# blepping/ComfyUI-sonar

Measured on AMD Instinct MI355X. Metric: noise-latents/sec (SDXL 4x128x128), higher is better.
Workload: dtype f32

## Files before the change

comfyui-sonar_amd/csrc/plan.hip:

```cpp
#include <math.h>
#include <string.h>

#include <memory>
#include <type_traits>
#include <utility>
#include <vector>

#include "common.h"

namespace sonar {
namespace {

template <typename T>
inline T word_to(uint64_t w) {
    if constexpr (std::is_pointer_v<T>) {
        return reinterpret_cast<T>(static_cast<uintptr_t>(w));
    } else if constexpr (std::is_same_v<T, float>) {
        const uint32_t lo = (uint32_t)w;
        float f;
        memcpy(&f, &lo, sizeof f);
        return f;
    } else if constexpr (std::is_same_v<T, double>) {
        double d;
        memcpy(&d, &w, sizeof d);
// ... 42 lines not shown
    SONAR_REPLAYABLE(sonar_philox_normal_chain_f32),
    SONAR_REPLAYABLE(sonar_perlin_lattice_f32),
    SONAR_REPLAYABLE(sonar_perlin_generate_f32),
    SONAR_REPLAYABLE(sonar_perlin_generate_acc_f32),
    SONAR_REPLAYABLE(sonar_perlin_generate_chain_f32),
    SONAR_REPLAYABLE(sonar_perlin_noise_f32),
    SONAR_REPLAYABLE(sonar_perlin_noise_ahead_f32),
    SONAR_REPLAYABLE(sonar_pyramid_generate_f32),
    SONAR_REPLAYABLE(sonar_pyramid_generate_acc_f32),
    SONAR_REPLAYABLE(sonar_pyramid_generate_acc_ahead_f32),
    SONAR_REPLAYABLE(sonar_pyramid_noise_f32),
    SONAR_REPLAYABLE(sonar_pyramid_noise_ahead_f32),
    SONAR_REPLAYABLE(sonar_power_noise_f32),
    SONAR_REPLAYABLE(sonar_power_block_f32),
    SONAR_REPLAYABLE(sonar_power_noise_ahead_f32),
    SONAR_REPLAYABLE(sonar_power_irfft2_f32),
    SONAR_REPLAYABLE(sonar_spectral_filter_f32),
    SONAR_REPLAYABLE(sonar_channel_mix_f32),
    SONAR_REPLAYABLE(sonar_std_scale_f32),
    SONAR_REPLAYABLE(sonar_powerlaw_f32),
    SONAR_REPLAYABLE(sonar_mul_table_f32),
    SONAR_REPLAYABLE(sonar_stats_finalize),
    SONAR_REPLAYABLE(sonar_scale_noise_rows_f32),
    SONAR_REPLAYABLE(sonar_blend_f32),
    SONAR_REPLAYABLE(sonar_blend_tensor_f32),
    SONAR_REPLAYABLE(sonar_scalar_op_f32),
    SONAR_REPLAYABLE(sonar_rowstats_f32),
    SONAR_REPLAYABLE(sonar_row_affine_f32),
    SONAR_REPLAYABLE(sonar_amax_mid_f32),
    SONAR_REPLAYABLE(sonar_div_mid_f32),
// ... 208 lines not shown
```

comfyui-sonar_amd/csrc/power_core.h:

```cpp
#pragma once
#include <math.h>
#include <stdlib.h>

#include <type_traits>

#include "common.h"
#include "twiddles256.h"

namespace sonar {

using c32 = float2;

typedef float v2f __attribute__((ext_vector_type(2)));
__device__ __forceinline__ v2f vv(c32 a) { return v2f{a.x, a.y}; }
__device__ __forceinline__ c32 cc(v2f a) { return make_float2(a.x, a.y); }
__device__ __forceinline__ c32 cadd(c32 a, c32 b) { return cc(vv(a) + vv(b)); }
__device__ __forceinline__ c32 csub(c32 a, c32 b) { return cc(vv(a) - vv(b)); }
__device__ __forceinline__ c32 cmul(c32 a, c32 b) {
    const v2f A = vv(a), B = vv(b);
    return cc(__builtin_elementwise_fma(A.yy, v2f{-B.y, B.x}, A.xx * B));
}
__device__ __forceinline__ c32 cadd_i(c32 a, c32 b) { return cc(__builtin_elementwise_fma(vv(b).yx, v2f{-1.0f, 1.0f}, vv(a))); }
__device__ __forceinline__ c32 csub_i(c32 a, c32 b) { return cc(__builtin_elementwise_fma(vv(b).yx, v2f{1.0f, -1.0f}, vv(a))); }
__device__ __forceinline__ c32 cmul_i(c32 a) { return cc(vv(a).yx * v2f{-1.0f, 1.0f}); }
// ... 292 lines not shown
constexpr int kStatsBatch = 4;
struct StatsAhead {
    double* partials = nullptr;
    uint64_t stream_id = 0;
    int main_blocks = 0;
};
template <int H, int W>
__device__ __forceinline__ void power_stats_body(const float* __restrict__ filter, int64_t planes, uint64_t seed, uint64_t stream_id,
                                                 int64_t plane_offset, int group, int split, double* partials, int64_t bid, int64_t nb,
                                                 c32 (*EDGE)[2][H], double* red);

struct Ahead {
    int have_stats = 0;
    uint64_t next_stream = 0;
    double* next = nullptr;
};


}
```

comfyui-sonar_amd/csrc/power_fft.hip:

```cpp
#include "power_core.h"

namespace sonar {

template <int H, int W>
constexpr int plane_min_waves() {
    return (H * W >= 32768 || (H == 256 && W == 64) || (H == 64 && W == 256) || (H == 64 && W == 32)) ? 2 : 4;
}

template <int H, int W, int SRC, bool STATS, bool NORM>
__global__ void __launch_bounds__((plane_threads<H, W>()), (plane_min_waves<H, W>())) power_irfft2_kernel(const float* __restrict__ z,
                                                                       const float* __restrict__ filter, float* out,
                                                                       int64_t planes, uint64_t seed, uint64_t stream_id,
                                                                       int64_t plane_offset, int group, int split, double* partials,
                                                                       NormArgs na, StatsAhead sa) {
    kernarg_touch_for(z, filter, out, planes, seed, stream_id, plane_offset, group, split, partials, na, sa);
    using C = PlaneCfg<H, W>;
    constexpr int NT = plane_threads<H, W>();
    constexpr int M = C::M, S = C::S;
    constexpr int RN1 = C::RN1, RN2 = C::RN2;
    constexpr bool FAST = (W == 128) && (H == 128 || H == 64) && (NT == 512);
    constexpr int CN1 = FAST ? H / 8 : C::CN1, CN2 = FAST ? 8 : C::CN2;
    __shared__ c32 A[C::kLdsComplex];
    c32* const T0 = A + H * S;
    c32* const TM = T0 + H;
// ... 1021 lines not shown
            }
            partials_next[2 * slot] = ss;
            partials_next[2 * slot + 1] = qq;
        }
    }
};

template <int IT0, int IT1, int N>
__device__ __forceinline__ void pin_chunk(c32 (&v)[N]) {
#pragma unroll
    for (int it = IT0; it < IT1; ++it) {
        asm volatile("" : "+v"(v[it].x), "+v"(v[it].y), "+v"(v[it + N / 2].x), "+v"(v[it + N / 2].y));
    }
}

template <int H, int W, bool STATS, bool NORM>
__global__ void __launch_bounds__(1024) power_pipe_kernel(const float* __restrict__ filter, float* out, int64_t planes, uint64_t seed,
                                                          uint64_t stream_id, int64_t plane_offset, int group, int split, double* partials,
                                                          NormArgs na, uint64_t next_stream, double* partials_next) {
    kernarg_touch_for(filter, out, planes, seed, stream_id, plane_offset, group, split, partials, na, next_stream, partials_next);
    using C = PlaneCfg<H, W>;
    constexpr int NT = 512, NALL = 1024;
    static_assert(plane_threads<H, W>() == NT && W == 128 && H == 128, "one 8-wave team per plane, slot = one radix-16 column item");
    constexpr int M = C::M, S = C::S, Wh = M + 1, RN1 = C::RN1, RN2 = C::RN2, CN1 = H / 8, CN2 = 8, ITER = draw_iters<H, W>();
    constexpr int LM = draw_shift<W>();
    constexpr int E0 = kPipeChunks[0], E1 = E0 + kPipeChunks[1];
    static_assert(E1 <= ITER && ITER == CN1 / 2, "chunks of whole pair iterations");
    constexpr int BUF = H * S;
    __shared__ c32 PLANES[2 * BUF];
    __shared__ c32 EDGE[3 * H];
    __shared__ uint4 SEED_RT[NT];
    static_assert(sizeof(uint4) * NT >= sizeof(c32) * 2 * H * kAheadMaxGroup, "edge columns of a look-ahead unit fit the seed area");
    __shared__ double sred[2 * NT / 64];
    __shared__ double red[2 * NALL / 64];
// ... 245 lines not shown
                    gp = 0;
                    unit += gridDim.x;
                }
            }
            SONAR_PIPE_STAMP(3);
            __syncthreads();
        }
    }
    if (ahead) {
        __syncthreads();
        if (drawer && my_units == 2) TeamStats<H, W>::store(sred, tid, partials_next, (int64_t)blockIdx.x + gridDim.x);
    }
    if constexpr (STATS) write_partial<NALL>(s, q, partials, red);
}

template <int H, int W>
__device__ __forceinline__ void power_stats_body(const float* __restrict__ filter, int64_t planes, uint64_t seed, uint64_t stream_id,
                                                 int64_t plane_offset, int group, int split, double* partials, int64_t bid, int64_t nb,
                                                 c32 (*EDGE)[2][H] , double* red) {
    constexpr int NT = plane_threads<H, W>(), M = W / 2, Wh = M + 1;
    constexpr int NB = kStatsBatch;
    const int tid = threadIdx.x;
    double s = 0.0, q = 0.0;
    auto edge_terms = [&](int p) {
        float edge = 0.0f;
        for (int ky = tid; ky < H; ky += NT) {
            const int kn = (H - ky) & (H - 1);
            const c32 a = EDGE[p][0][ky], an = EDGE[p][0][kn], b = EDGE[p][1][ky], bn = EDGE[p][1][kn];
            const float ar = 0.5f * (a.x + an.x), ai = 0.5f * (a.y - an.y), br = 0.5f * (b.x + bn.x), bi = 0.5f * (b.y - bn.y);
            edge += (ar * ar + ai * ai) + (br * br + bi * bi);
// ... 86 lines not shown
template <int H, int W>
static int power_grid(int64_t planes, bool owns_partials = true) {
    using C = PlaneCfg<H, W>;
    static_assert(C::kLdsBytes + 256 <= 160 * 1024, "plane does not fit in LDS");
    const int threads_cu = H >= 128 ? 1024 : 2048;
    const int per_cu = (int)std::max<size_t>(1, std::min<size_t>(threads_cu / plane_threads<H, W>(), (160 * 1024) / (C::kLdsBytes + 256)));
    const int64_t g = std::min<int64_t>(planes, (int64_t)256 * per_cu);
    return (int)(owns_partials ? std::min<int64_t>(g, kNPart) : g);
}

static int& pipe_switch() {
    static int on = [] { const char* e = getenv("SONAR_POWER_PIPE"); return (e && e[0] == '0') ? 0 : 1; }();
    return on;
}
static bool pipe_enabled() { return pipe_switch() != 0; }
static int64_t pipe_units(int64_t planes, int group, int* psplit) {
    *psplit = group > 1 && planes / group < 256 ? 1 : 0;
    return *psplit ? planes : planes / group;
}

template <int H, int W>
static int launch_power(int what, const float* z, const float* filter, float* out, int64_t planes, uint64_t seed,
                        uint64_t stream_id, int64_t plane_offset, int group, double* partials, NormArgs na, hipStream_t st,
                        Ahead ah = Ahead()) {
    if constexpr (H == 128 && W == 128) {
        if (pipe_enabled() && z == nullptr && (what == 0 || what == 1) && planes > 256) {
            int psplit;
            const int64_t units = pipe_units(planes, group, &psplit);
            const int pg = (int)std::min<int64_t>(units, 256);
            if (what == 1) {
                if (!ah.have_stats)
                    hipLaunchKernelGGL((power_stats_kernel<H, W>), dim3(std::min<int64_t>(units, kNPart)), dim3(plane_threads<H, W>()), 0, st, filter,
                                       planes, seed, stream_id, plane_offset, group, psplit, partials);
                hipLaunchKernelGGL((power_pipe_kernel<H, W, false, true>), dim3(pg), dim3(1024), 0, st, filter, out, planes, seed, stream_id,
                                   plane_offset, group, psplit, (double*)nullptr, na, ah.next_stream, ah.next);
            } else if (partials) {
                hipLaunchKernelGGL((power_pipe_kernel<H, W, true, false>), dim3(pg), dim3(1024), 0, st, filter, out, planes, seed, stream_id,
                                   plane_offset, group, psplit, partials, na, (uint64_t)0, (double*)nullptr);
            } else {
                hipLaunchKernelGGL((power_pipe_kernel<H, W, false, false>), dim3(pg), dim3(1024), 0, st, filter, out, planes, seed, stream_id,
                                   plane_offset, group, psplit, partials, na, (uint64_t)0, (double*)nullptr);
            }
            return check_launch("sonar_power_*");
        }
    }
    const int split = group > 1 && planes / group < 2 * 256 ? 1 : 0;
    const int64_t ngroups = split ? planes : planes / group;
    const dim3 blk(plane_threads<H, W>());
#define SONAR_PW(G, ST, NM, PART) \
    hipLaunchKernelGGL((power_irfft2_kernel<H, W, G, ST, NM>), dim3(power_grid<H, W>(ngroups, ST)), blk, 0, st, z, filter, out, planes, seed, stream_id, plane_offset, group, split, PART, na, StatsAhead())
    if (what == 4) {
        SONAR_PW(3, false, false, nullptr);
    } else if (what == 3) {
        if constexpr (H == 128 && W == 128) {
            const dim3 grid(power_grid<H, W>(planes, partials != nullptr));
            if (partials) hipLaunchKernelGGL((spectral_filter128_kernel<H, W, true>), grid, blk, 0, st, z, filter, out, planes, partials);
// ... 200 lines not shown
    SONAR_REQUIRE(filter && out && partials && planes >= 0 && H > 0 && W > 0 && plane_offset >= 0, SONAR_ERR_ARG,
                  "sonar_power_noise_ahead_f32: bad argument");
    SONAR_REQUIRE((reinterpret_cast<uintptr_t>(out) & 7u) == 0 && partials_next != partials, SONAR_ERR_ARG,
                  "sonar_power_noise_ahead_f32: misaligned buffer, or the same workspace for both calls' statistics");
    SONAR_REQUIRE(sonar_power_noise_ahead_ok(planes, H, W, rng_group), SONAR_ERR_UNSUPPORTED,
                  "sonar_power_noise_ahead_f32: no look-ahead for %lld planes of %lld x %lld (ask sonar_power_noise_ahead_ok first)", (long long)planes,
                  (long long)H, (long long)W);
    Ahead ah;
    ah.have_stats = have_stats != 0;
    ah.next_stream = next_stream_id;
    ah.next = partials_next;
    return power_dispatch(1, nullptr, filter, out, planes, H, W, seed, stream_id, plane_offset, rng_group, partials,
                          NormArgs{partials, planes * H * W, factor, threshold_std_devs}, (hipStream_t)stream, ah);
}

extern "C" int sonar_spectral_filter_f32(const float* x, const float* filter, float* out, int64_t planes, int64_t H, int64_t W,
                                         double* partials, void* stream) {
    SONAR_REQUIRE(x && filter && out && x != out && planes >= 0 && H > 0 && W > 0, SONAR_ERR_ARG,
                  "sonar_spectral_filter_f32: bad argument (in-place not supported)");
    SONAR_REQUIRE((reinterpret_cast<uintptr_t>(out) & 7u) == 0 && (reinterpret_cast<uintptr_t>(x) & 7u) == 0, SONAR_ERR_ARG,
                  "sonar_spectral_filter_f32: misaligned buffer");
    if (planes == 0) return SONAR_OK;
    return power_dispatch(3, x, filter, out, planes, H, W, 0, 0, 0, 1, partials, NormArgs{nullptr, 0, 1.0f, 0.0f}, (hipStream_t)stream);
}

extern "C" int sonar_rfft2_f32(const float* x, float* z_out, int64_t planes, int64_t H, int64_t W, void* stream) {
    SONAR_REQUIRE(x && z_out && planes >= 0 && H > 0 && W > 0, SONAR_ERR_ARG, "sonar_rfft2_f32: bad argument");
    SONAR_REQUIRE((reinterpret_cast<uintptr_t>(z_out) & 7u) == 0 && (reinterpret_cast<uintptr_t>(x) & 7u) == 0, SONAR_ERR_ARG,
                  "sonar_rfft2_f32: misaligned buffer");
    if (planes == 0) return SONAR_OK;
// ... 27 lines not shown
```

comfyui-sonar_amd/hip_lib.py:

```python
from __future__ import annotations

import ctypes as C
import math
import os
import threading as _threading
import weakref
from typing import Optional, Sequence

import torch

_HERE = os.path.dirname(os.path.abspath(__file__))
LIB_PATH = os.path.join(_HERE, "libsonar_hip.so")

BLEND_IDS = {"lerp": 0, "inject": 1, "subtract_b": 2}
MODE_IDS = {"CLASSIC": 0, "NEW": 1, "DENOISED": 2}
INIT_IDS = {"NONE": 0, "SAMPLE": 1, "SAMPLE_NORM": 2}
RESAMPLE_IDS = {"bilinear": 0, "nearest-exact": 1, "area": 2, "adaptive_avg_pool2d": 2, "nearest": 3, "bicubic": 4, "bicubic_aligned": 5,
                "bilinear_aligned": 6}
UPSCALE_MODES = ("bilinear", "nearest-exact", "area", "adaptive_avg_pool2d", "nearest", "bicubic")
PYRAMID_FUSED_MODES = ("bilinear", "nearest-exact", "area", "adaptive_avg_pool2d")
DWT_MODE_IDS = {"zero": 0, "symmetric": 1, "reflect": 2, "periodization": 3, "periodic": 4, "constant": 5, "replicate": 5}
NPART = 1024
BROWNIAN_MAX_TERMS = 96
ERR_ARG, ERR_UNSUPPORTED, ERR_HIP = -1, -2, -3
# ... 92 lines not shown
    "sonar_perlin_noise_f32": (_I, [_P, _P, _I64, _I64, _I64, _F, _U64, _U64, _I64, _F, _F, _P, _P]),
    "sonar_perlin_noise_ahead_ok": (_I, [_I64, _I64, _I64]),
    "sonar_perlin_noise_ahead_f32": (_I, [_P, _P, _I64, _I64, _F, _U64, _U64, _I64, _F, _F, _P, _I, _U64, _P, _P, _P, _I64, _I64, _I64, _I64, _I, _U64, _P]),
    "sonar_resample_acc_f32": (_I, [_P, _P, _I64, _I64, _I64, _I64, _I64, _F, _I, _I, _P, _P]),
    "sonar_pyramid_generate_f32": (_I, [_P, _I64, _I64, _I64, _I64, C.POINTER(_P), _PI64, _PI64, _PF, _I, _U64, _U64, _I64, _P, _P]),
    "sonar_pyramid_noise_f32": (_I, [_P, _I64, _I64, _I64, _I64, C.POINTER(_P), _PI64, _PI64, _PF, _I, _U64, _U64, _I64, _F, _F, _P, _P]),
    "sonar_pyramid_noise_ahead_f32": (_I, [_P, _I64, _I64, _I64, _I64, _PI64, _PI64, _PF, _I, _U64, _U64, _I64, _F, _F, _P, _I, _U64, _I64, _PI64, _PI64, _PF, _P,
                                           _P]),
    "sonar_levels_sampled_f32": (_I, [_P, _I64, _I64, _I64, _I, _PI64, _PI64, _PF, _PF, _I, _U64, _U64, _I64, _I, _P]),
    "sonar_level_normal_f32": (_I, [_P, _I64, _I64, _I64, _F, _U64, _U64, _I64, _P]),
    "sonar_power_noise_f32": (_I, [_P, _P, _I64, _I64, _I64, _U64, _U64, _I64, _I, _F, _F, _P, _P]),
    "sonar_power_noise_ahead_ok": (_I, [_I64, _I64, _I64, _I]),
    "sonar_power_pipeline": (_I, [_I]),
    "sonar_wcfg_hi_storage": (_I, [_I]),
    "sonar_power_noise_ahead_f32": (_I, [_P, _P, _I64, _I64, _I64, _U64, _U64, _I64, _I, _F, _F, _P, _I, _U64, _P, _P]),
    "sonar_power_spectrum_f32": (_I, [_P, _I64, _I64, _I64, _U64, _U64, _I64, _I, _P]),
    "sonar_power_irfft2_f32": (_I, [_P, _P, _P, _I64, _I64, _I64, _U64, _U64, _I64, _I, _P, _P]),
    "sonar_spectral_filter_f32": (_I, [_P, _P, _P, _I64, _I64, _I64, _P, _P]),
    "sonar_std_scale_f32": (_I, [_P, _I64, _F, _P, _I64, _I64, _P]),
    "sonar_channel_mix_f32": (_I, [_P, _P, _P, _I64, _I64, _I64, _P, _P]),
    "sonar_dwt_out_len": (_I64, [_I64, _I64, _I]),
    "sonar_dwt2_ws_bytes": (_I64, [_I64, _I64, _I64, _I, _I, _I, _I]),
    "sonar_dwt2_fwd_f32": (_I, [_P, _P, _P, _I64, _I64, _I64, _PD, _PD, _I, _I, _P, _P]),
    "sonar_dwt2_fwd_f64": (_I, [_P, _P, _P, _I64, _I64, _I64, _PD, _PD, _I, _I, _P, _P]),
    "sonar_dwt2_inv_f32": (_I, [_P, _I64, _I64, _P, _P, _I64, _I64, _I64, _I64, _I64, _PD, _PD, _I, _I, _P, _P]),
    "sonar_dwt2_inv_f64": (_I, [_P, _I64, _I64, _P, _P, _I64, _I64, _I64, _I64, _I64, _PD, _PD, _I, _I, _P, _P]),
    "sonar_sq_acc_f32": (_I, [_P, _P, _F, _I, _I64, _P]),
    "sonar_studentt_f32": (_I, [_P, _P, _F, _F, _F, _I64, _P]),
    "sonar_abs_quantile_rows_f32": (_I, [_P, _I64, _I64, _I64, _F, _P, _P]),
    "sonar_clamp_signpow_rows_f32": (_I, [_P, _I64, _I64, _P, _F, _F, _P]),
# ... 962 lines not shown
    if kind in (3, 4):
        if z is None:
            white = philox_normal(tuple(shape), filt.device, seed, stream_id, plane_offset * H * W)
            return _direct_spectral_filter(white, filt, partials)
        return _direct_inverse(z, filt, out, 1.0 / math.sqrt(H * W), partials)
    _check(
        load().sonar_power_irfft2_f32(zp, _dev(filt, "filter"), _dev(out, "out"), planes, H, W, seed & (2**64 - 1), stream_id, plane_offset,
                                      rng_group_for(shape), _opt(partials, "partials", torch.float64), _stream()),
        "sonar_power_irfft2_f32",
    )
    return out


class PowerLookahead:

    __slots__ = ("key", "partials", "last_stream", "last_delta", "step", "hits", "misses")

    def __init__(self):
        self.key = None
        self.partials = None
        self.last_stream = None
        self.last_delta = None
        self.step = 1
        self.hits = 0
        self.misses = 0


def power_noise(filt: torch.Tensor, shape, *, seed: int, stream_id: int, plane_offset: int, factor: float,
                threshold_std_devs: float = 2.5, lookahead: Optional[PowerLookahead] = None) -> torch.Tensor:
    H, W = shape[-2:]
    out = torch.empty(shape, dtype=torch.float32, device=filt.device)
    planes = out.numel() // (H * W)
    kind = power_plane_kind(H, W)
    if kind == 4:
        return _power_block(1, filt, out, seed, stream_id, plane_offset, partials=new_partials(filt.device), factor=factor,
# ... 8 lines not shown
    if lookahead is not None and lib.sonar_power_noise_ahead_ok(planes, H, W, group):
        st = _stream()

        def key_for(stream, seed=seed, st=st):
            return (filt.data_ptr(), filt._version, tuple(shape), seed, stream, plane_offset, group, filt.device, st)

        have = lookahead.key is not None and lookahead.key == key_for(stream_id)
        ws = lookahead.partials if have else new_partials(filt.device)
        if lookahead.last_stream is not None and stream_id > lookahead.last_stream:
            delta = stream_id - lookahead.last_stream
            if lookahead.last_delta is None or delta == lookahead.last_delta:
                lookahead.step = delta
            lookahead.last_delta = delta
        nxt = (stream_id + lookahead.step) & (2**64 - 1)
        nws = new_partials(filt.device)
        _check(
            lib.sonar_power_noise_ahead_f32(_dev(filt, "filter"), _dev(out, "out"), planes, H, W, seed, stream_id, plane_offset, group,
                                            float(factor), float(threshold_std_devs), _dev(ws, "ws", torch.float64), int(have), nxt,
                                            _dev(nws, "ws_next", torch.float64), st),
            "sonar_power_noise_ahead_f32",
        )
        lookahead.hits += int(have)
        lookahead.misses += int(not have)
        lookahead.key, lookahead.partials, lookahead.last_stream = key_for(nxt), nws, stream_id
        rec = _recorder
        if rec is not None and rec.thread == _threading.get_ident():
            if have and lookahead.last_delta == lookahead.step:
                rec.hooks.append(_PowerAheadHook(lookahead, key_for, ws, nws, stream_id - rec.base, lookahead.step, filt.device))
            else:
                rec.fail("power-law look-ahead not in its steady state")
        return out
    ws = new_partials(filt.device)
    _check(
        lib.sonar_power_noise_f32(_dev(filt, "filter"), _dev(out, "out"), planes, H, W, seed, stream_id, plane_offset,
                                  group, float(factor), float(threshold_std_devs), _dev(ws, "ws", torch.float64), _stream()),
        "sonar_power_noise_f32",
    )
    return out


def spectral_filter(x: torch.Tensor, filt: torch.Tensor, partials: Optional[torch.Tensor] = None) -> torch.Tensor:
    H, W = int(x.shape[-2]), int(x.shape[-1])
    planes = x.numel() // (H * W)
# ... 595 lines not shown
        return out


def wcfg_fused(cond: torch.Tensor, uncond: torch.Tensor, x: Optional[torch.Tensor], **params):
    return FusedCall(**params)(cond, uncond, x)


PLANS_ENABLED = os.environ.get("SONAR_PLANS", "1") != "0"
PLAN_WARM_CALLS = 2
PLAN_MAX_ATTEMPTS = 3
FILL_AHEAD = os.environ.get("SONAR_FILL_AHEAD", "1") != "0"
PYRAMID_AHEAD = os.environ.get("SONAR_PYRAMID_AHEAD", "1") != "0"
PERLIN_AHEAD = os.environ.get("SONAR_PERLIN_AHEAD", "1") != "0"
NOT_RUN = object()
_M64 = 2**64 - 1
_HOST_QUERIES = frozenset(("sonar_abi_version", "sonar_noise_stream_version", "sonar_last_error", "sonar_noise_params_ws_doubles", "sonar_group_stats_ws_doubles", "sonar_power_noise_ahead_ok", "sonar_perlin_noise_ahead_ok", "sonar_philox_noise_ahead_ok", "sonar_power_pipeline", "sonar_wcfg_hi_storage", "sonar_power_plane_kind", "sonar_dwt_out_len",
                           "sonar_dwt2_ws_bytes", "sonar_wcfg_lowpass_lds_bytes", "sonar_wcfg_fused_ws_bytes", "sonar_pyramid_levels",
                           "sonar_plan_fn_id", "sonar_plan_fn_nargs"))
PATCH_SLOT, PATCH_STREAM, PATCH_SEED, PATCH_BLOB, PATCH_LEVELS = range(5)


class PlanPatch(C.Structure):

    _fields_ = [("source", C.c_int32), ("target", C.c_int32), ("index", C.c_int32), ("width", C.c_int32), ("addend", C.c_int64)]


class PlanLevels(C.Structure):

    _fields_ = [("H", C.c_int64), ("W", C.c_int64), ("discount", C.c_double), ("iterations", C.c_int32), ("reserved", C.c_int32),
                ("h_offset", C.c_int64), ("w_offset", C.c_int64), ("weight_offset", C.c_int64)]

# ... 73 lines not shown

def load_raw() -> C.CDLL:
    return _lib if _lib is not None else load()


class PlanHook:

    managed: dict = {}

    def bind(self, slot_of: dict):
        pass


class _PowerAheadHook(PlanHook):

    def __init__(self, la, key_for, ws, nws, rel: int, step: int, device):
        self.la, self.key_for, self.rel, self.step, self.device = la, key_for, rel, step, device
        self.managed = {ws.data_ptr(): "ws", nws.data_ptr(): "nws"}
        self.pair = None
        self.flip = 0

    def bind(self, slot_of):
        self.ws_slot, self.nws_slot = slot_of["ws"], slot_of["nws"]

    def pre_run(self, seed, base, table, st):
        la = self.la
        stream = base + self.rel
        if (la.key is None or la.step != self.step or la.last_stream is None or stream - la.last_stream != self.step
                or la.key != self.key_for(stream, seed, st)):
            return None
        if self.pair is None:
            self.pair = (new_partials(self.device), new_partials(self.device))
        nws = self.pair[self.flip]
        if nws is la.partials:
            self.flip ^= 1
            nws = self.pair[self.flip]
        table[self.ws_slot] = la.partials.data_ptr()
        table[self.nws_slot] = nws.data_ptr()
        return stream, seed, st, nws

    def post_run(self, token):
        stream, seed, st, nws = token
        la = self.la
        la.hits += 1
        la.key, la.partials, la.last_stream, la.last_delta = self.key_for((stream + self.step) & _M64, seed, st), nws, stream, self.step
        self.flip ^= 1


class _AheadHook(PlanHook):

    KEYS = ()
    BUFFERS = (0, 0)

    def __init__(self, count: int, device, *, sa: int = 0, la: int = 0, lattice=None):
        self.count, self.device = count, device
        self.sa, self.la, self.lattice = sa, la, lattice
        self.by_stream = {}
        self.hits = self.misses = 0

    def _state(self, st: int):
# ... 699 lines not shown
```

include/sonar_hip.h:

```cpp
#ifndef SONAR_HIP_H
#define SONAR_HIP_H

#include <stdint.h>

#ifdef __cplusplus
extern "C" {
#endif

#define SONAR_OK 0
#define SONAR_ERR_ARG (-1)
#define SONAR_ERR_UNSUPPORTED (-2)
#define SONAR_ERR_HIP (-3)

#define SONAR_BLEND_LERP 0
#define SONAR_BLEND_INJECT 1
#define SONAR_BLEND_SUBTRACT_B 2

#define SONAR_MODE_CLASSIC 0
#define SONAR_MODE_NEW 1
#define SONAR_MODE_DENOISED 2

#define SONAR_INIT_NONE 0
#define SONAR_INIT_SAMPLE 1
#define SONAR_INIT_SAMPLE_NORM 2
// ... 310 lines not shown
int sonar_power_block_f32(const float* filter, float* ws, float* out, int64_t planes, int64_t H, int64_t W, uint64_t seed, uint64_t stream_id,
                          int64_t plane_offset, int rng_group, int mode, float factor, float threshold_std_devs, double* partials ,
                          void* stream);
int sonar_power_irfft2_f32(const float* z, const float* filter, float* out, int64_t planes, int64_t H, int64_t W,
                           uint64_t seed, uint64_t stream_id, int64_t plane_offset, int rng_group,
                           double* partials , void* stream);
int sonar_power_noise_f32(const float* filter, float* out, int64_t planes, int64_t H, int64_t W, uint64_t seed,
                          uint64_t stream_id, int64_t plane_offset, int rng_group, float factor, float threshold_std_devs,
                          double* partials , void* stream);

int sonar_power_noise_ahead_ok(int64_t planes, int64_t H, int64_t W, int rng_group);
int sonar_power_pipeline(int enable);
int sonar_power_noise_ahead_f32(const float* filter, float* out, int64_t planes, int64_t H, int64_t W, uint64_t seed,
                                uint64_t stream_id, int64_t plane_offset, int rng_group, float factor, float threshold_std_devs,
                                double* partials, int have_stats, uint64_t next_stream_id, double* partials_next, void* stream);
int sonar_power_spectrum_f32(float* z_out, int64_t planes, int64_t H, int64_t W, uint64_t seed, uint64_t stream_id,
                             int64_t plane_offset, int rng_group, void* stream);
int sonar_spectral_filter_f32(const float* x, const float* filter, float* out, int64_t planes, int64_t H, int64_t W,
                              double* partials, void* stream);
int sonar_std_scale_f32(float* x, int64_t n, float mul, const double* partials, int64_t npart, int64_t n_total, void* stream);
int sonar_channel_mix_f32(const float* in, const float* mixer, float* out, int64_t B, int64_t C, int64_t hw,
                          double* partials , void* stream);

int64_t sonar_dwt_out_len(int64_t n, int64_t flen, int mode);
int64_t sonar_dwt2_ws_bytes(int64_t planes, int64_t H, int64_t W, int flen, int mode, int elem_size, int inverse);
int sonar_dwt2_fwd_f32(const float* x, float* ll, float* hi, int64_t planes, int64_t H, int64_t W,
                       const double* dec_lo, const double* dec_hi, int flen, int mode, void* ws, void* stream);
int sonar_dwt2_fwd_f64(const double* x, double* ll, double* hi, int64_t planes, int64_t H, int64_t W,
                       const double* dec_lo, const double* dec_hi, int flen, int mode, void* ws, void* stream);
int sonar_dwt2_inv_f32(const float* ll, int64_t ll_h, int64_t ll_w, const float* hi, float* out, int64_t planes,
// ... 110 lines not shown
```

Before: 12.67 million.

## Carry first plane's column pass and RNG state across power-noise calls

Adds a carry variant of the pipelined power-law noise kernel. Each block computes the first spectrum draw and column IDFT of the next call's first plane and stores it, along with its RNG states, in a per-block global workspace. The next call loads that state into LDS instead of starting with a cold draw-only step, which removes the pipeline fill at kernel start. The cost is extra global writes and reads per block and more host bookkeeping (carry keys, plan-replay hooks), and the carry is only used when the look-ahead is in its steady state.

```diff
diff --git a/comfyui-sonar_amd/csrc/plan.hip b/comfyui-sonar_amd/csrc/plan.hip
--- a/comfyui-sonar_amd/csrc/plan.hip
+++ b/comfyui-sonar_amd/csrc/plan.hip
@@ -80,6 +80,7 @@
     SONAR_REPLAYABLE(sonar_power_noise_f32),
     SONAR_REPLAYABLE(sonar_power_block_f32),
     SONAR_REPLAYABLE(sonar_power_noise_ahead_f32),
+    SONAR_REPLAYABLE(sonar_power_noise_carry_f32),
     SONAR_REPLAYABLE(sonar_power_irfft2_f32),
     SONAR_REPLAYABLE(sonar_spectral_filter_f32),
     SONAR_REPLAYABLE(sonar_channel_mix_f32),
diff --git a/comfyui-sonar_amd/csrc/power_core.h b/comfyui-sonar_amd/csrc/power_core.h
--- a/comfyui-sonar_amd/csrc/power_core.h
+++ b/comfyui-sonar_amd/csrc/power_core.h
@@ -330,7 +330,9 @@
     int have_stats = 0;
     uint64_t next_stream = 0;
     double* next = nullptr;
-};
-
-
-}
+    float* carry_ws = nullptr;
+    int carry_in = 0, carry_out = 0;
+};
+
+
+}
diff --git a/comfyui-sonar_amd/csrc/power_fft.hip b/comfyui-sonar_amd/csrc/power_fft.hip
--- a/comfyui-sonar_amd/csrc/power_fft.hip
+++ b/comfyui-sonar_amd/csrc/power_fft.hip
@@ -1059,10 +1059,20 @@
     }
 }
 
-template <int H, int W, bool STATS, bool NORM>
+struct PipeCarry {
+    float* ws;
+    int in, out;
+};
+template <int H, int W>
+constexpr int64_t pipe_carry_slot_bytes() {
+    return (int64_t)sizeof(c32) * H * PlaneCfg<H, W>::S + (int64_t)sizeof(uint4) * plane_threads<H, W>() + (int64_t)sizeof(uint2) * H;
+}
+
+template <int H, int W, bool STATS, bool NORM, bool CARRY = false>
 __global__ void __launch_bounds__(1024) power_pipe_kernel(const float* __restrict__ filter, float* out, int64_t planes, uint64_t seed,
                                                           uint64_t stream_id, int64_t plane_offset, int group, int split, double* partials,
-                                                          NormArgs na, uint64_t next_stream, double* partials_next) {
+                                                          NormArgs na, uint64_t next_stream, double* partials_next, PipeCarry) {
+    static_assert(!CARRY, "the carry form is a specialisation of its own (below)");
     kernarg_touch_for(filter, out, planes, seed, stream_id, plane_offset, group, split, partials, na, next_stream, partials_next);
     using C = PlaneCfg<H, W>;
     constexpr int NT = 512, NALL = 1024;
@@ -1338,6 +1348,357 @@
     if constexpr (STATS) write_partial<NALL>(s, q, partials, red);
 }
 
+template <>
+__global__ void __launch_bounds__(1024) power_pipe_kernel<128, 128, false, true, true>(const float* __restrict__ filter, float* out, int64_t planes,
+                                                                                     uint64_t seed, uint64_t stream_id, int64_t plane_offset,
+                                                                                     int group, int split, double* partials, NormArgs na,
+                                                                                     uint64_t next_stream, double* partials_next, PipeCarry cy) {
+    kernarg_touch_for(filter, out, planes, seed, stream_id, plane_offset, group, split, partials, na, next_stream, partials_next, cy);
+    constexpr int H = 128, W = 128;
+    constexpr bool STATS = false, NORM = true;
+    using C = PlaneCfg<H, W>;
+    constexpr int NT = 512, NALL = 1024;
+    constexpr int M = C::M, S = C::S, Wh = M + 1, CN1 = H / 8, CN2 = 8, ITER = draw_iters<H, W>();
+    constexpr int LM = draw_shift<W>();
+    constexpr int E0 = kPipeChunks[0], E1 = E0 + kPipeChunks[1];
+    constexpr int BUF = H * S;
+    static_assert(plane_threads<H, W>() == NT && E1 <= ITER && ITER == CN1 / 2 && BUF % 2 == 0 && kNPart == NALL, "as the kernel above");
+    __shared__ c32 PLANES[2 * BUF];
+    __shared__ c32 EDGE[3 * H];
+    __shared__ uint4 SEED_RT[NT];
+    __shared__ uint4 NEXT_RT[NT];
+    __shared__ uint2 SEED_E[H], NEXT_E[H];
+    static_assert(sizeof(uint4) * NT >= sizeof(c32) * 2 * H * kAheadMaxGroup, "edge columns of a look-ahead unit fit the seed area");
+    static_assert(sizeof(PLANES) + sizeof(EDGE) + sizeof(SEED_RT) + sizeof(NEXT_RT) + sizeof(SEED_E) + sizeof(NEXT_E) + 1024 <= 160 * 1024, "LDS");
+    __shared__ double sred[2][2 * NT / 64];
+    __shared__ double red[2 * NALL / 64];
+    __shared__ NormDecision shd;
+    const int wv_all = __builtin_amdgcn_readfirstlane((int)threadIdx.x >> 6);
+    const bool drawer = wv_all >= NT / 64;
+    const int tid = threadIdx.x & (NT - 1), lane = threadIdx.x & 63, wv = wv_all & (NT / 64 - 1);
+    const int64_t nunits = split ? planes : planes / group;
+    const int64_t group0 = plane_offset / group;
+    const int per_unit = split ? 1 : group;
+    const int64_t my_units = (int64_t)blockIdx.x < nunits ? (nunits - blockIdx.x + gridDim.x - 1) / gridDim.x : 0;
+    const int n = (int)(my_units * per_unit);
+    const bool ahead = partials_next != nullptr && nunits <= 2 * (int64_t)gridDim.x;
+    const bool cin = cy.in != 0 && n > 0, cout = cy.out != 0 && n > 0;
+    char* const slot = reinterpret_cast<char*>(cy.ws) + (int64_t)blockIdx.x * pipe_carry_slot_bytes<H, W>();
+    c32* const slot_plane = reinterpret_cast<c32*>(slot);
+    uint4* const slot_rt = reinterpret_cast<uint4*>(slot + sizeof(c32) * BUF);
+    uint2* const slot_e = reinterpret_cast<uint2*>(slot + sizeof(c32) * BUF + sizeof(uint4) * NT);
+    const float scale = 1.0f / sqrtf((float)H * (float)W);
+    float nm = scale, nc = 0.0f;
+    double pre_s = na.partials[2 * threadIdx.x], pre_q = na.partials[2 * threadIdx.x + 1];
+    auto carry_to_lds = [&]() {
+        constexpr int CPY = (BUF / 2 + NALL - 1) / NALL;
+        float4 cpy[CPY];
+#pragma unroll
+        for (int i = 0; i < CPY; ++i) {
+            const int e = (int)threadIdx.x + i * NALL;
+            if (e < BUF / 2) cpy[i] = reinterpret_cast<const float4*>(slot_plane)[e];
+        }
+#pragma unroll
+        for (int i = 0; i < CPY; ++i) {
+            const int e = (int)threadIdx.x + i * NALL;
+            if (e < BUF / 2) {
+                PLANES[2 * e] = make_float2(cpy[i].x, cpy[i].y);
+                PLANES[2 * e + 1] = make_float2(cpy[i].z, cpy[i].w);
+            }
+        }
+    };
+    auto leave_wave_sums = [&]() {
+        const double ws = wave_sum(pre_s), wq = wave_sum(pre_q);
+        if (lane == 0) {
+            red[wv_all] = ws;
+            red[NALL / 64 + wv_all] = wq;
+        }
+    };
+    auto decide_in_wave0 = [&]() {
+        if (wv_all == 0) {
+            double ss = 0.0, qq = 0.0;
+#pragma unroll
+            for (int i = 0; i < NALL / 64; ++i) {
+                ss += red[i];
+                qq += red[NALL / 64 + i];
+            }
+            const NormDecision dec = decision_from_totals(ss, qq, na.n_total, na.thr_sd);
+            if (lane == 0) shd = dec;
+        }
+    };
+    auto pick_up_decision = [&]() {
+        const NormDecision dec = shd;
+        const float g = (dec.do_div ? 1.0f / dec.stdv : 1.0f) * na.factor;
+        nm = scale * g;
+        nc = dec.do_sub ? dec.mean * g : 0.0f;
+    };
+    double s = 0.0, q = 0.0;
+    if (drawer) {
+        __builtin_amdgcn_s_setprio(kPipePrioDraw);
+        const c32* const Q = EDGE + 2 * H;
+        SpectrumRng rng;
+        uint4 rt_in = make_uint4(0, 1, 0, 1);
+        if (cin) rt_in = slot_rt[tid];
+        float wa[ITER], wb[ITER];
+        bool neg = false;
+#pragma unroll
+        for (int it = 0; it < ITER; ++it) {
+            const int p = tid + it * NT, pos = (p >> LM) * Wh + 1 + (p & (M - 1));
+            const float fa = filter[pos], fb = filter[pos + (H / 2) * Wh];
+            wa[it] = filter_weight(fa);
+            wb[it] = filter_weight(fb);
+            neg = neg || fa < 0.0f || fb < 0.0f;
+        }
+        const bool wave_neg = __builtin_amdgcn_ballot_w64(neg) != 0;
+        c32 ctw[CN1];
+#pragma unroll
+        for (int k1 = 0; k1 < CN1; ++k1) ctw[k1] = c_tw256[((wv * k1) * (256 / H)) & 255];
+        const int col = (lane + 1) & (M - 1);
+        int64_t unit = blockIdx.x;
+        int gp = 0;
+        auto seed_next = [&]() {
+            const GroupWalk gw(blockIdx.x, group, split);
+            SpectrumRng g = spectrum_rng<H, true>(seed, next_stream, group0 + gw.grp, tid);
+            for (int i = 0; i < gw.first; ++i) skip_plane<H, W, true>(g, tid);
+            NEXT_RT[tid] = make_uint4(g.R.x, g.R.c, g.T.x, g.T.c);
+            if (tid < H) NEXT_E[tid] = make_uint2(g.E.x, g.E.c);
+        };
+        if (cin) {
+            rng.R = Mwc{rt_in.x, rt_in.y};
+            rng.T = Mwc{rt_in.z, rt_in.w};
+            if (per_unit == 1) unit += gridDim.x;
+            else gp = 1;
+            if (n == 1 && cout) seed_next();
+            carry_to_lds();
+            leave_wave_sums();
+            __syncthreads();
+        }
+        for (int j = cin ? 1 : 0; j <= n; ++j) {
+            const bool carry = j == n;
+            SONAR_PIPE_STAMP(0);
+            if (carry && !cout) {
+                SONAR_PIPE_STAMP(1);
+                __syncthreads();
+                SONAR_PIPE_STAMP(2);
+                __syncthreads();
+                SONAR_PIPE_STAMP(3);
+                __syncthreads();
+                break;
+            }
+            c32* const A = PLANES + (j & 1) * BUF;
+            c32 v[CN1];
+            if (carry) {
+                const uint4 rt = NEXT_RT[tid];
+                rng.R = Mwc{rt.x, rt.y};
+                rng.T = Mwc{rt.z, rt.w};
+            } else if (gp == 0 && !(cin && j == 1)) {
+                const GroupWalk gw(unit, group, split);
+                if (j == per_unit) {
+                    const uint4 rt = SEED_RT[tid];
+                    rng.R = Mwc{rt.x, rt.y};
+                    rng.T = Mwc{rt.z, rt.w};
+                } else {
+                    rng = spectrum_seed<true>(seed, stream_id, group0 + gw.grp, tid, false);
+                }
+                for (int i = 0; i < gw.first; ++i) skip_plane<H, W, true, false>(rng, tid);
+            }
+            draw_chunk_regs<H, W, 0, E0>(rng, v, wa, wb);
+            if (wave_neg) draw_chunk_signs<H, W, 0, E0>(filter, tid, v);
+            pin_chunk<0, E0>(v);
+            if (j == (cin ? 1 : 0) && n > per_unit && !(cin && per_unit == 1)) {
+                const GroupWalk gw((int64_t)blockIdx.x + gridDim.x, group, split);
+                const SpectrumRng g2 = spectrum_rng<H, true>(seed, stream_id, group0 + gw.grp, tid);
+                SEED_RT[tid] = make_uint4(g2.R.x, g2.R.c, g2.T.x, g2.T.c);
+                if (tid < H) SEED_E[tid] = make_uint2(g2.E.x, g2.E.c);
+            }
+            if (j == n - 1 && cout) seed_next();
+            if (carry && per_unit == 1 && n > 1) {
+                const GroupWalk gw((int64_t)blockIdx.x + gridDim.x, group, split);
+                SpectrumRng g = spectrum_rng<H, true>(seed, next_stream, group0 + gw.grp, tid);
+                for (int i = 0; i < gw.first; ++i) skip_plane<H, W, true>(g, tid);
+                slot_rt[tid] = make_uint4(g.R.x, g.R.c, g.T.x, g.T.c);
+                if (tid < H) slot_e[tid] = make_uint2(g.E.x, g.E.c);
+            }
+            SONAR_PIPE_STAMP(1);
+            __syncthreads();
+            draw_chunk_regs<H, W, E0, E1>(rng, v, wa, wb);
+            if (wave_neg) draw_chunk_signs<H, W, E0, E1>(filter, tid, v);
+            pin_chunk<E0, E1>(v);
+            SONAR_PIPE_STAMP(2);
+            __syncthreads();
+            draw_chunk_regs<H, W, E1, ITER>(rng, v, wa, wb);
+            if (wave_neg) draw_chunk_signs<H, W, E1, ITER>(filter, tid, v);
+            if (lane == M - 1) {
+#pragma unroll
+                for (int n1 = 0; n1 < CN1; ++n1) v[n1] = Q[CN2 * n1 + wv];
+            }
+            idft<CN1>(v);
+#pragma unroll
+            for (int k1 = 1; k1 < CN1; ++k1) v[k1] = cmul(v[k1], ctw[k1]);
+            if (carry) {
+                int coff = col;
+                asm volatile("" : "+v"(coff));
+#pragma unroll
+                for (int k1 = 0; k1 < CN1; ++k1) (slot_plane + (CN2 * k1 + wv) * S)[coff] = v[k1];
+                if (per_unit > 1) slot_rt[tid] = make_uint4(rng.R.x, rng.R.c, rng.T.x, rng.T.c);
+            } else {
+#pragma unroll
+                for (int k1 = 0; k1 < CN1; ++k1) A[(CN2 * k1 + wv) * S + col] = v[k1];
+                if (++gp == per_unit) {
+                    gp = 0;
+                    unit += gridDim.x;
+                }
+            }
+            if (j == 0) leave_wave_sums();
+            SONAR_PIPE_STAMP(3);
+            __syncthreads();
+        }
+        if (ahead) {
+            [[maybe_unused]] const int j = n + 1;
+            const bool mine = my_units == 2;
+            SONAR_PIPE_STAMP(0);
+            TeamStats<H, W> ts;
+            c32* const edge = reinterpret_cast<c32*>(SEED_RT);
+            if (mine) {
+                const GroupWalk gw((int64_t)blockIdx.x + gridDim.x, group, split);
+                ts.begin(filter, seed, next_stream, plane_offset, group, gw, tid, edge, wa, wb);
+                ts.radii(0, 4, tid);
+                ts.products();
+            }
+            SONAR_PIPE_STAMP(1);
+            __syncthreads();
+            if (mine) ts.edges_and_wave_sums(edge, tid, sred[1]);
+            SONAR_PIPE_STAMP(2);
+            __syncthreads();
+            if (mine) TeamStats<H, W>::store(sred[1], tid, partials_next, (int64_t)blockIdx.x + gridDim.x);
+            SONAR_PIPE_STAMP(3);
+        }
+    } else {
+        __builtin_amdgcn_s_setprio(kPipePrioFft);
+        int64_t unit = blockIdx.x;
+        int gp = 0;
+        c32* const T0 = EDGE;
+        c32* const TM = EDGE + H;
+        c32* const Q = EDGE + 2 * H;
+        const float f0 = tid < H ? filter[tid * Wh] : 0.0f, fm = tid < H ? filter[tid * Wh + M] : 0.0f;
+        Mwc rngE{0, 1};
+        int64_t eunit = blockIdx.x;
+        int egp = 0;
+        auto draw_edges = [&](int je) {
+            if (tid < H && (je < n || (je == n && cout))) {
+                if (je == n) {
+                    const uint2 e = NEXT_E[tid];
+                    rngE = Mwc{e.x, e.y};
+                } else if (egp == 0 && !(cin && je == 1)) {
+                    const GroupWalk gw(eunit, group, split);
+                    if (je == per_unit) {
+                        const uint2 e = SEED_E[tid];
+                        rngE = Mwc{e.x, e.y};
+                    } else {
+                        rngE = spectrum_seed<false>(seed, stream_id, group0 + gw.grp, tid, true).E;
+                    }
+                    for (int i = 0; i < 3 * gw.first; ++i) rngE.next();
+                }
+                const uint32_t r0 = rngE.next();
+                const uint32_t rm = rngE.next();
+                const uint32_t t = rngE.next();
+                T0[tid] = drawn_elem(r0, angle_lo(t), f0);
+                TM[tid] = drawn_elem(rm, angle_hi(t), fm);
+                if (je == n) {
+                    if (per_unit > 1) slot_e[tid] = make_uint2(rngE.x, rngE.c);
+                } else if (++egp == per_unit) {
+                    egp = 0;
+                    eunit += gridDim.x;
+                }
+            }
+        };
+        auto pack_edges = [&](int je) {
+            if (tid >= NT - H && (je < n || (je == n && cout))) {
+                const int ky = tid - (NT - H), kn = (H - ky) & (H - 1);
+                const c32 a = T0[ky], an = T0[kn], b = TM[ky], bn = TM[kn];
+                Q[ky] = make_float2(0.5f * (a.x + an.x) - 0.5f * (b.y - bn.y), 0.5f * (a.y - an.y) + 0.5f * (b.x + bn.x));
+            }
+        };
+        auto exchange = [] { __syncthreads(); };
+        if (cin) {
+            if (tid < H) {
+                const uint2 e = slot_e[tid];
+                rngE = Mwc{e.x, e.y};
+            }
+            if (per_unit == 1) eunit += gridDim.x;
+            else egp = 1;
+            carry_to_lds();
+            leave_wave_sums();
+            __syncthreads();
+        } else {
+            [[maybe_unused]] const int j = 0;
+            SONAR_PIPE_STAMP(0);
+            draw_edges(0);
+            SONAR_PIPE_STAMP(1);
+            exchange();
+            pack_edges(0);
+            SONAR_PIPE_STAMP(2);
+            exchange();
+            leave_wave_sums();
+            SONAR_PIPE_STAMP(3);
+            __syncthreads();
+        }
+        for (int j = 1; j <= n; ++j) {
+            constexpr int NW = 8;
+            c32* const X = PLANES + ((j + 1) & 1) * BUF;
+            c32* const Y = PLANES + (j & 1) * BUF;
+            SONAR_PIPE_STAMP(0);
+            pipe_col_b<H, W, NW>(X, Y, wv, lane);
+            draw_edges(j);
+            if (j == 1) decide_in_wave0();
+            SONAR_PIPE_STAMP(1);
+            exchange();
+            pipe_row_a<H, W, NW>(Y, X, wv, lane);
+            pack_edges(j);
+            SONAR_PIPE_STAMP(2);
+            exchange();
+            {
+                if (j == 1) pick_up_decision();
+                const GroupWalk gw(unit, group, split);
+                float* const oplane = out + (gw.grp * group + gw.first + gp) * (int64_t)H * W;
+                pipe_row_b<H, W, NW, STATS, NORM>(X, oplane, wv, lane, scale, nm, nc, s, q);
+                if (++gp == per_unit) {
+                    gp = 0;
+                    unit += gridDim.x;
+                }
+            }
+            SONAR_PIPE_STAMP(3);
+            __syncthreads();
+        }
+        if (ahead) {
+            [[maybe_unused]] const int j = n + 1;
+            const bool mine = my_units >= 1;
+            __builtin_amdgcn_s_setprio(kPipePrioDraw);
+            SONAR_PIPE_STAMP(0);
+            TeamStats<H, W> ts;
+            c32* const edge = PLANES + BUF;
+            if (blockIdx.x == 0)
+                for (int64_t sl = nunits + tid; sl < kNPart; sl += NT) {
+                    partials_next[2 * sl] = 0.0;
+                    partials_next[2 * sl + 1] = 0.0;
+                }
+            if (mine) {
+                const GroupWalk gw(blockIdx.x, group, split);
+                ts.begin(filter, seed, next_stream, plane_offset, group, gw, tid, edge);
+                ts.radii(0, 4, tid);
+                ts.products();
+            }
+            SONAR_PIPE_STAMP(1);
+            __syncthreads();
+            if (mine) ts.edges_and_wave_sums(edge, tid, sred[0]);
+            SONAR_PIPE_STAMP(2);
+            __syncthreads();
+            if (mine) TeamStats<H, W>::store(sred[0], tid, partials_next, blockIdx.x);
+            SONAR_PIPE_STAMP(3);
+        }
+    }
+}
+
 template <int H, int W>
 __device__ __forceinline__ void power_stats_body(const float* __restrict__ filter, int64_t planes, uint64_t seed, uint64_t stream_id,
                                                  int64_t plane_offset, int group, int split, double* partials, int64_t bid, int64_t nb,
@@ -1454,6 +1815,10 @@
     return on;
 }
 static bool pipe_enabled() { return pipe_switch() != 0; }
+static int& carry_switch() {
+    static int on = [] { const char* e = getenv("SONAR_POWER_CARRY"); return (e && e[0] == '1') ? 1 : 0; }();
+    return on;
+}
 static int64_t pipe_units(int64_t planes, int group, int* psplit) {
     *psplit = group > 1 && planes / group < 256 ? 1 : 0;
     return *psplit ? planes : planes / group;
@@ -1472,14 +1837,19 @@
                 if (!ah.have_stats)
                     hipLaunchKernelGGL((power_stats_kernel<H, W>), dim3(std::min<int64_t>(units, kNPart)), dim3(plane_threads<H, W>()), 0, st, filter,
                                        planes, seed, stream_id, plane_offset, group, psplit, partials);
-                hipLaunchKernelGGL((power_pipe_kernel<H, W, false, true>), dim3(pg), dim3(1024), 0, st, filter, out, planes, seed, stream_id,
-                                   plane_offset, group, psplit, (double*)nullptr, na, ah.next_stream, ah.next);
+                if (ah.carry_ws && (ah.carry_in || ah.carry_out))
+                    hipLaunchKernelGGL((power_pipe_kernel<H, W, false, true, true>), dim3(pg), dim3(1024), 0, st, filter, out, planes, seed,
+                                       stream_id, plane_offset, group, psplit, (double*)nullptr, na, ah.next_stream, ah.next,
+                                       PipeCarry{ah.carry_ws, ah.carry_in, ah.carry_out});
+                else
+                    hipLaunchKernelGGL((power_pipe_kernel<H, W, false, true>), dim3(pg), dim3(1024), 0, st, filter, out, planes, seed, stream_id,
+                                       plane_offset, group, psplit, (double*)nullptr, na, ah.next_stream, ah.next, PipeCarry{});
             } else if (partials) {
                 hipLaunchKernelGGL((power_pipe_kernel<H, W, true, false>), dim3(pg), dim3(1024), 0, st, filter, out, planes, seed, stream_id,
-                                   plane_offset, group, psplit, partials, na, (uint64_t)0, (double*)nullptr);
+                                   plane_offset, group, psplit, partials, na, (uint64_t)0, (double*)nullptr, PipeCarry{});
             } else {
                 hipLaunchKernelGGL((power_pipe_kernel<H, W, false, false>), dim3(pg), dim3(1024), 0, st, filter, out, planes, seed, stream_id,
-                                   plane_offset, group, psplit, partials, na, (uint64_t)0, (double*)nullptr);
+                                   plane_offset, group, psplit, partials, na, (uint64_t)0, (double*)nullptr, PipeCarry{});
             }
             return check_launch("sonar_power_*");
         }
@@ -1710,6 +2080,45 @@
                           NormArgs{partials, planes * H * W, factor, threshold_std_devs}, (hipStream_t)stream, ah);
 }
 
+extern "C" int sonar_power_carry(int enable) {
+    const int before = carry_switch();
+    if (enable >= 0) carry_switch() = enable != 0;
+    return before;
+}
+
+extern "C" int64_t sonar_power_noise_carry_ws_bytes(int64_t planes, int64_t H, int64_t W, int rng_group) {
+    if (!carry_switch() || H != 128 || W != 128 || !pipe_enabled() || planes <= 256 || !sonar_power_noise_ahead_ok(planes, H, W, rng_group)) return 0;
+    return 256 * pipe_carry_slot_bytes<128, 128>();
+}
+
+extern "C" int sonar_power_noise_carry_f32(const float* filter, float* out, int64_t planes, int64_t H, int64_t W, uint64_t seed,
+                                           uint64_t stream_id, int64_t plane_offset, int rng_group, float factor,
+                                           float threshold_std_devs, double* partials, int have_stats, uint64_t next_stream_id,
+                                           double* partials_next, float* carry_ws, int carry_in, int carry_out, void* stream) {
+    SONAR_REQUIRE(filter && out && partials && planes >= 0 && H > 0 && W > 0 && plane_offset >= 0, SONAR_ERR_ARG,
+                  "sonar_power_noise_carry_f32: bad argument");
+    SONAR_REQUIRE((reinterpret_cast<uintptr_t>(out) & 7u) == 0 && partials_next != partials && (reinterpret_cast<uintptr_t>(carry_ws) & 15u) == 0,
+                  SONAR_ERR_ARG, "sonar_power_noise_carry_f32: misaligned buffer, or the same workspace for both calls' statistics");
+    SONAR_REQUIRE(sonar_power_noise_ahead_ok(planes, H, W, rng_group), SONAR_ERR_UNSUPPORTED,
+                  "sonar_power_noise_carry_f32: no look-ahead for %lld planes of %lld x %lld (ask sonar_power_noise_ahead_ok first)", (long long)planes,
+                  (long long)H, (long long)W);
+    const bool carry = carry_ws != nullptr && (carry_in != 0 || carry_out != 0);
+    SONAR_REQUIRE(!carry || sonar_power_noise_carry_ws_bytes(planes, H, W, rng_group) > 0, SONAR_ERR_UNSUPPORTED,
+                  "sonar_power_noise_carry_f32: no carried plane for %lld planes of %lld x %lld (sonar_power_noise_carry_ws_bytes says 0)",
+                  (long long)planes, (long long)H, (long long)W);
+    Ahead ah;
+    ah.have_stats = have_stats != 0;
+    ah.next_stream = next_stream_id;
+    ah.next = partials_next;
+    if (carry) {
+        ah.carry_ws = carry_ws;
+        ah.carry_in = carry_in != 0;
+        ah.carry_out = carry_out != 0;
+    }
+    return power_dispatch(1, nullptr, filter, out, planes, H, W, seed, stream_id, plane_offset, rng_group, partials,
+                          NormArgs{partials, planes * H * W, factor, threshold_std_devs}, (hipStream_t)stream, ah);
+}
+
 extern "C" int sonar_spectral_filter_f32(const float* x, const float* filter, float* out, int64_t planes, int64_t H, int64_t W,
                                          double* partials, void* stream) {
     SONAR_REQUIRE(x && filter && out && x != out && planes >= 0 && H > 0 && W > 0, SONAR_ERR_ARG,
diff --git a/comfyui-sonar_amd/hip_lib.py b/comfyui-sonar_amd/hip_lib.py
--- a/comfyui-sonar_amd/hip_lib.py
+++ b/comfyui-sonar_amd/hip_lib.py
@@ -130,6 +130,9 @@
     "sonar_power_pipeline": (_I, [_I]),
     "sonar_wcfg_hi_storage": (_I, [_I]),
     "sonar_power_noise_ahead_f32": (_I, [_P, _P, _I64, _I64, _I64, _U64, _U64, _I64, _I, _F, _F, _P, _I, _U64, _P, _P]),
+    "sonar_power_noise_carry_ws_bytes": (_I64, [_I64, _I64, _I64, _I]),
+    "sonar_power_carry": (_I, [_I]),
+    "sonar_power_noise_carry_f32": (_I, [_P, _P, _I64, _I64, _I64, _U64, _U64, _I64, _I, _F, _F, _P, _I, _U64, _P, _P, _I, _I, _P]),
     "sonar_power_spectrum_f32": (_I, [_P, _I64, _I64, _I64, _U64, _U64, _I64, _I, _P]),
     "sonar_power_irfft2_f32": (_I, [_P, _P, _P, _I64, _I64, _I64, _U64, _U64, _I64, _I, _P, _P]),
     "sonar_spectral_filter_f32": (_I, [_P, _P, _P, _I64, _I64, _I64, _P, _P]),
@@ -1122,11 +1125,13 @@
 
 class PowerLookahead:
 
-    __slots__ = ("key", "partials", "last_stream", "last_delta", "step", "hits", "misses")
+    __slots__ = ("key", "partials", "last_stream", "last_delta", "step", "hits", "misses", "carry", "carry_key")
 
     def __init__(self):
         self.key = None
         self.partials = None
+        self.carry = None
+        self.carry_key = None
         self.last_stream = None
         self.last_delta = None
         self.step = 1
@@ -1165,19 +1170,36 @@
             lookahead.last_delta = delta
         nxt = (stream_id + lookahead.step) & (2**64 - 1)
         nws = new_partials(filt.device)
-        _check(
-            lib.sonar_power_noise_ahead_f32(_dev(filt, "filter"), _dev(out, "out"), planes, H, W, seed, stream_id, plane_offset, group,
-                                            float(factor), float(threshold_std_devs), _dev(ws, "ws", torch.float64), int(have), nxt,
-                                            _dev(nws, "ws_next", torch.float64), st),
-            "sonar_power_noise_ahead_f32",
-        )
+        cbytes = lib.sonar_power_noise_carry_ws_bytes(planes, H, W, group)
+        carry = None
+        if cbytes > 0:
+            carry = lookahead.carry
+            if carry is None or carry.numel() < cbytes or carry.device != filt.device:
+                carry = lookahead.carry = torch.empty(cbytes, dtype=torch.uint8, device=filt.device)
+                lookahead.carry_key = None
+            carry_in = have and lookahead.carry_key == lookahead.key
+            _check(
+                lib.sonar_power_noise_carry_f32(_dev(filt, "filter"), _dev(out, "out"), planes, H, W, seed, stream_id, plane_offset, group,
+                                                float(factor), float(threshold_std_devs), _dev(ws, "ws", torch.float64), int(have), nxt,
+                                                _dev(nws, "ws_next", torch.float64), _dev(carry, "carry_ws", torch.uint8), int(carry_in), 1, st),
+                "sonar_power_noise_carry_f32",
+            )
+        else:
+            carry_in = False
+            _check(
+                lib.sonar_power_noise_ahead_f32(_dev(filt, "filter"), _dev(out, "out"), planes, H, W, seed, stream_id, plane_offset, group,
+                                                float(factor), float(threshold_std_devs), _dev(ws, "ws", torch.float64), int(have), nxt,
+                                                _dev(nws, "ws_next", torch.float64), st),
+                "sonar_power_noise_ahead_f32",
+            )
         lookahead.hits += int(have)
         lookahead.misses += int(not have)
         lookahead.key, lookahead.partials, lookahead.last_stream = key_for(nxt), nws, stream_id
+        lookahead.carry_key = lookahead.key if carry is not None else None
         rec = _recorder
         if rec is not None and rec.thread == _threading.get_ident():
-            if have and lookahead.last_delta == lookahead.step:
-                rec.hooks.append(_PowerAheadHook(lookahead, key_for, ws, nws, stream_id - rec.base, lookahead.step, filt.device))
+            if have and lookahead.last_delta == lookahead.step and (carry is None or carry_in):
+                rec.hooks.append(_PowerAheadHook(lookahead, key_for, ws, nws, stream_id - rec.base, lookahead.step, filt.device, carry))
             else:
                 rec.fail("power-law look-ahead not in its steady state")
         return out
@@ -1803,7 +1825,7 @@
 PERLIN_AHEAD = os.environ.get("SONAR_PERLIN_AHEAD", "1") != "0"
 NOT_RUN = object()
 _M64 = 2**64 - 1
-_HOST_QUERIES = frozenset(("sonar_abi_version", "sonar_noise_stream_version", "sonar_last_error", "sonar_noise_params_ws_doubles", "sonar_group_stats_ws_doubles", "sonar_power_noise_ahead_ok", "sonar_perlin_noise_ahead_ok", "sonar_philox_noise_ahead_ok", "sonar_power_pipeline", "sonar_wcfg_hi_storage", "sonar_power_plane_kind", "sonar_dwt_out_len",
+_HOST_QUERIES = frozenset(("sonar_abi_version", "sonar_noise_stream_version", "sonar_last_error", "sonar_noise_params_ws_doubles", "sonar_group_stats_ws_doubles", "sonar_power_noise_ahead_ok", "sonar_perlin_noise_ahead_ok", "sonar_philox_noise_ahead_ok", "sonar_power_pipeline", "sonar_power_carry", "sonar_power_noise_carry_ws_bytes", "sonar_wcfg_hi_storage", "sonar_power_plane_kind", "sonar_dwt_out_len",
                            "sonar_dwt2_ws_bytes", "sonar_wcfg_lowpass_lds_bytes", "sonar_wcfg_fused_ws_bytes", "sonar_pyramid_levels",
                            "sonar_plan_fn_id", "sonar_plan_fn_nargs"))
 PATCH_SLOT, PATCH_STREAM, PATCH_SEED, PATCH_BLOB, PATCH_LEVELS = range(5)
@@ -1907,20 +1929,26 @@
 
 class _PowerAheadHook(PlanHook):
 
-    def __init__(self, la, key_for, ws, nws, rel: int, step: int, device):
+    def __init__(self, la, key_for, ws, nws, rel: int, step: int, device, carry=None):
         self.la, self.key_for, self.rel, self.step, self.device = la, key_for, rel, step, device
         self.managed = {ws.data_ptr(): "ws", nws.data_ptr(): "nws"}
+        self.carries = carry is not None
+        if self.carries:
+            self.managed[carry.data_ptr()] = "carry"
         self.pair = None
         self.flip = 0
 
     def bind(self, slot_of):
         self.ws_slot, self.nws_slot = slot_of["ws"], slot_of["nws"]
+        self.carry_slot = slot_of["carry"] if self.carries else None
 
     def pre_run(self, seed, base, table, st):
         la = self.la
         stream = base + self.rel
         if (la.key is None or la.step != self.step or la.last_stream is None or stream - la.last_stream != self.step
                 or la.key != self.key_for(stream, seed, st)):
+            return None
+        if self.carries and (la.carry is None or la.carry_key != la.key):
             return None
         if self.pair is None:
             self.pair = (new_partials(self.device), new_partials(self.device))
@@ -1930,6 +1958,8 @@
             nws = self.pair[self.flip]
         table[self.ws_slot] = la.partials.data_ptr()
         table[self.nws_slot] = nws.data_ptr()
+        if self.carries:
+            table[self.carry_slot] = la.carry.data_ptr()
         return stream, seed, st, nws
 
     def post_run(self, token):
@@ -1937,6 +1967,7 @@
         la = self.la
         la.hits += 1
         la.key, la.partials, la.last_stream, la.last_delta = self.key_for((stream + self.step) & _M64, seed, st), nws, stream, self.step
+        la.carry_key = la.key if self.carries else None
         self.flip ^= 1
 
 
diff --git a/include/sonar_hip.h b/include/sonar_hip.h
--- a/include/sonar_hip.h
+++ b/include/sonar_hip.h
@@ -348,6 +348,12 @@
 int sonar_power_noise_ahead_f32(const float* filter, float* out, int64_t planes, int64_t H, int64_t W, uint64_t seed,
                                 uint64_t stream_id, int64_t plane_offset, int rng_group, float factor, float threshold_std_devs,
                                 double* partials, int have_stats, uint64_t next_stream_id, double* partials_next, void* stream);
+int64_t sonar_power_noise_carry_ws_bytes(int64_t planes, int64_t H, int64_t W, int rng_group);
+int sonar_power_carry(int enable);
+int sonar_power_noise_carry_f32(const float* filter, float* out, int64_t planes, int64_t H, int64_t W, uint64_t seed,
+                                uint64_t stream_id, int64_t plane_offset, int rng_group, float factor, float threshold_std_devs,
+                                double* partials, int have_stats, uint64_t next_stream_id, double* partials_next, float* carry_ws,
+                                int carry_in, int carry_out, void* stream);
 int sonar_power_spectrum_f32(float* z_out, int64_t planes, int64_t H, int64_t W, uint64_t seed, uint64_t stream_id,
                              int64_t plane_offset, int rng_group, void* stream);
 int sonar_spectral_filter_f32(const float* x, const float* filter, float* out, int64_t planes, int64_t H, int64_t W,
```

After: 12.70 million, median of 2. No clear change (+0.2%).
